# mmaker/c-lwe-snarks

Hardware: AMD Instinct MI355X
Metric: snark_proofs_per_sec (higher is better)
Workload: dtype u32 limbs (704-bit integers mod 2^704) + AES-256 bytes; int8 digits on the matrix cores, int32 accumulation (exact)

## Files before the change

### c-lwe-snarks_amd/__init__.py

```python
from __future__ import annotations

import ctypes
import os
from dataclasses import dataclass

import numpy as np

_HERE = os.path.dirname(os.path.abspath(__file__))
LIB_PATH = os.environ.get("MFHIP_LIB") or os.path.join(_HERE, "libmfhip.so")
P = 0xFFFFFFFB


class MfhError(RuntimeError):
    pass


@dataclass(frozen=True)
class Params:

    n: int = 1470
    logq: int = 736
    d: int = 1 << 15
    m: int = 21845

# ... 34 lines not shown
        return 2 * self.ctr_ct * self.d + self.ctr_ct

    @property
    def ct_limbs(self):
        return (self.n + 1) * self.L


DEBUG = Params(d=256, m=64)
DEFAULT = Params()


class _CParams(ctypes.Structure):
    _fields_ = [("n", ctypes.c_uint32), ("logq", ctypes.c_uint32), ("d", ctypes.c_uint32), ("m", ctypes.c_uint32)]


_lib = None

EXPORTS = [
    "mfh_ctx_create", "mfh_ctx_destroy", "mfh_set_stream", "mfh_sync", "mfh_scrub_staging", "mfh_last_error", "mfh_set_seed",
    "mfh_keystream", "mfh_sample_rows", "mfh_ct_add", "mfh_ct_mul_ui", "mfh_ct_addmul_ui", "mfh_eval_rows",
    "mfh_encrypt_rows", "mfh_decrypt", "mfh_ct_smudge", "mfh_ssp_upload", "mfh_witness_poly", "mfh_version",
    "mfh_workspace_bytes", "mfh_last_kernel_ms", "mfh_set_timing", "mfh_set_overlap", "mfh_eval_rows_multi", "mfh_prove_batch", "mfh_crs_mm_image_bytes", "mfh_crs_expand_mm", "mfh_crs_set_resident_mm", "mfh_witness_poly_multi", "mfh_witness_poly_mm", "mfh_poly_h_multi", "mfh_poly_mul", "mfh_poly_add", "mfh_poly_prepare_t",
    "mfh_ssp_prepare", "mfh_poly_h", "mfh_setup_messages", "mfh_setup", "mfh_setup_image", "mfh_crs_image_set_b", "mfh_prove",
    "mfh_prove_partial", "mfh_prove_finish", "mfh_ct_to_lanes", "mfh_ct_from_lanes", "mfh_lanes_per_value", "mfh_digest128", "mfh_timing_drain", "mfh_timing_busy_ms", "mfh_timing_work_rows", "mfh_set_batch_image", "mfh_set_batch_slabs", "mfh_set_expand_path", "mfh_set_encrypt_path", "mfh_set_batch_launch", "mfh_set_batch_bw", "mfh_set_mm_chunk_rows", "mfh_set_mm_pack", "mfh_set_poly_exact", "mfh_poly_exact_fallbacks", "mfh_poly_exact_points", "mfh_set_poly_exact_points", "mfh_set_mm_stream", "mfh_add_dotp", "mfh_set_encrypt_chunks", "mfh_set_witness_per", "mfh_set_eval_path", "mfh_set_decrypt_path", "mfh_decrypt_rows",
    "mfh_crs_mm_share_bytes", "mfh_crs_expand_mm_share", "mfh_crs_set_resident_mm_share", "mfh_batch_chain", "mfh_batch_witness_cols", "mfh_batch_chain_from_w", "mfh_witness_poly_mm_cols", "mfh_prove_batch_partial", "mfh_prove_batch_finish",
    "mfh_resident_row_bytes", "mfh_crs_expand", "mfh_eval_rows_resident", "mfh_crs_set_resident",
    "mfh_witness_lanes", "mfh_witness_from_lanes", "mfh_prove_partial_w", "mfh_verify",
    "mfh_ssp_set_prg", "mfh_ssp_prg_make_t", "mfh_ssp_prg_fill",
    "mfh_resident_share_rows", "mfh_crs_expand_share", "mfh_crs_set_resident_share", "mfh_crs_set_resident_prefix",
    "mfh_prove_batch_supergroup", "mfh_prove_batch_stream_wait", "mfh_set_mm_width",
    "mfh_setup_public", "mfh_prove_public", "mfh_prove_batch_public", "mfh_vk_derive", "mfh_verify_public",
    "mfh_ssp_from_rows", "mfh_ssp_set_rows", "mfh_ssp_rows_fill", "mfh_circuit_create", "mfh_circuit_destroy", "mfh_circuit_assign",
    "mfh_circuit_create_global", "mfh_circuit_create_ex", "mfh_circuit_create_out", "mfh_circuit_create_sum",
]


def load_library():
    global _lib
    if _lib is not None:
        return _lib
    if not os.path.exists(LIB_PATH):
        raise MfhError(f"{LIB_PATH} is missing: run `python -c 'import __graft_entry__ as g; g.build()'` "
                       "(hipcc --offload-arch=gfx950).  There is no CPU fallback.")
    lib = ctypes.CDLL(LIB_PATH)
    vp, u64, sz, i32, u32 = ctypes.c_void_p, ctypes.c_uint64, ctypes.c_size_t, ctypes.c_int, ctypes.c_uint32
    sig = {
        "mfh_ctx_create": (i32, [ctypes.POINTER(vp), i32, ctypes.POINTER(_CParams)]),
# ... 58 lines not shown
        "mfh_witness_from_lanes": (i32, [vp, vp, vp, u32, vp]),
        "mfh_prove_partial_w": (i32, [vp, vp, vp, ctypes.c_char_p, u32, u32, u32, vp, vp]),
        "mfh_resident_row_bytes": (sz, [vp]),
        "mfh_crs_expand": (i32, [vp, u64, sz, vp, vp]),
        "mfh_crs_image_set_b": (i32, [vp, sz, sz, vp, vp]),
        "mfh_eval_rows_resident": (i32, [vp, vp, sz, sz, vp, vp, vp, vp, i32]),
        "mfh_crs_set_resident": (i32, [vp, vp]),
        "mfh_timing_drain": (i32, [vp, ctypes.c_char_p, ctypes.POINTER(u64), ctypes.POINTER(ctypes.c_double), ctypes.POINTER(u64),
                                   ctypes.POINTER(ctypes.c_float)]),
        "mfh_timing_busy_ms": (ctypes.c_double, [vp]),
        "mfh_timing_work_rows": (u64, [vp]),
        "mfh_set_batch_image": (i32, [vp, i32]),
        "mfh_set_mm_chunk_rows": (i32, [vp, u32]),
        "mfh_set_mm_pack": (i32, [vp, i32]),
        "mfh_set_poly_exact": (i32, [vp, i32]),
        "mfh_poly_exact_fallbacks": (ctypes.c_long, [vp]),
        "mfh_poly_exact_points": (i32, [vp, ctypes.POINTER(u32)]),
        "mfh_set_poly_exact_points": (i32, [vp, ctypes.POINTER(u32)]),
        "mfh_set_mm_stream": (i32, [vp, i32, i32, i32, u32]),
        "mfh_set_batch_launch": (i32, [vp, u32, i32]),
        "mfh_set_batch_bw": (i32, [vp, i32]),
        "mfh_set_encrypt_path": (i32, [vp, i32]),
        "mfh_set_expand_path": (i32, [vp, i32]),
        "mfh_set_batch_slabs": (i32, [vp, u32]),
        "mfh_set_encrypt_chunks": (i32, [vp, u32]),
        "mfh_set_eval_path": (i32, [vp, i32]),
        "mfh_set_decrypt_path": (i32, [vp, i32]),
        "mfh_decrypt_rows": (i32, [vp, u64, sz, vp, vp, vp]),
        "mfh_set_witness_per": (i32, [vp, u32]),
        "mfh_crs_mm_share_bytes": (sz, [vp, u32, u32]),
        "mfh_crs_expand_mm_share": (i32, [vp, vp, u32, u32, vp]),
        "mfh_crs_set_resident_mm_share": (i32, [vp, vp, u32, u32]),
        "mfh_batch_chain": (i32, [vp, vp, u32, ctypes.c_char_p, sz, vp, vp, vp, vp]),
        "mfh_batch_witness_cols": (i32, [vp, vp, u32, ctypes.c_char_p, sz, vp, u32, u32, vp, sz]),
        "mfh_batch_chain_from_w": (i32, [vp, vp, u32, vp, vp, vp]),
        "mfh_witness_poly_mm_cols": (i32, [vp, vp, u32, ctypes.c_char_p, sz, vp, u32, u32, vp, sz]),
        "mfh_prove_batch_partial": (i32, [vp, vp, u32, u32, u32, ctypes.c_char_p, sz, vp, vp, vp, sz, vp]),
        "mfh_prove_batch_finish": (i32, [vp, vp, u32, vp, ctypes.c_char_p, sz, ctypes.c_char_p, vp]),
        "mfh_setup_public": (i32, [vp, vp, u32, u32, u32, u32, vp, vp, vp, vp]),
        "mfh_prove_public": (i32, [vp, vp, vp, u32, ctypes.c_char_p, u32, ctypes.c_char_p, sz, ctypes.c_char_p, vp]),
        "mfh_prove_batch_public": (i32, [vp, vp, vp, u32, u32, ctypes.c_char_p, sz, vp, ctypes.c_char_p, sz, ctypes.c_char_p, vp]),
        "mfh_vk_derive": (i32, [vp, vp, u32, u32, vp]),
        "mfh_verify_public": (i32, [vp, vp, u32, u32, u32, vp, vp, ctypes.c_char_p, sz, sz, vp]),
        "mfh_ssp_from_rows": (i32, [vp, u32, vp, vp, vp, vp]),
        "mfh_ssp_set_rows": (i32, [vp, u32, vp, vp, vp, u32]),
        "mfh_ssp_rows_fill": (i32, [vp, sz, sz, vp]),
# ... 118 lines not shown
    def scrub_staging(self):
        rc = self.lib.mfh_scrub_staging(self._h)
        self._chk(rc)
        return rc

    def workspace_bytes(self):
        return int(self.lib.mfh_workspace_bytes(self._h))

    def set_timing(self, on=True):
        self._chk(self.lib.mfh_set_timing(self._h, 1 if on else 0))

    def set_overlap(self, mode=1):
        self._chk(self.lib.mfh_set_overlap(self._h, int(mode)))

    def set_batch_image(self, on=True):
        self._chk(self.lib.mfh_set_batch_image(self._h, 1 if on else 0))

    def set_batch_slabs(self, nslabs=0):
        self._chk(self.lib.mfh_set_batch_slabs(self._h, int(nslabs)))

    def set_expand_path(self, path=0):
        self._chk(self.lib.mfh_set_expand_path(self._h, int(path)))

    def set_encrypt_path(self, path=0):
        self._chk(self.lib.mfh_set_encrypt_path(self._h, int(path)))

    def set_eval_path(self, path=0):
        self._chk(self.lib.mfh_set_eval_path(self._h, int(path)))

    def set_encrypt_chunks(self, chunks=0):
        self._chk(self.lib.mfh_set_encrypt_chunks(self._h, int(chunks)))

    def set_witness_per(self, statements=0):
        self._chk(self.lib.mfh_set_witness_per(self._h, int(statements)))

    def set_batch_launch(self, groups_per_launch=4, merge_regions=True):
        self._chk(self.lib.mfh_set_batch_launch(self._h, int(groups_per_launch), 1 if merge_regions else 0))

    def set_batch_bw(self, merged=True):
        self._chk(self.lib.mfh_set_batch_bw(self._h, 1 if merged else 0))

    def set_mm_stream(self, map=0, persistent=False, sync_mode=0, spin_max=64):
        self._chk(self.lib.mfh_set_mm_stream(self._h, int(map), int(persistent), int(sync_mode), int(spin_max)))

    def set_mm_width(self, per_xcd=32, early_chain=False):
        self._chk(self.lib.mfh_set_mm_width(self._h, int(per_xcd), 1 if early_chain else 0))
# ... 494 lines not shown
```

### c-lwe-snarks_amd/csrc/ctx.hpp

```cpp
#pragma once
#include <hip/hip_runtime.h>

#include <stdint.h>
#include <string.h>

#include <string>
#include <vector>

#include "aes_dev.hpp"
#include "mfhip.h"
#include "ssp_prg.hpp"

#define HIP_TRY(ctx, expr)                                                        \
  do {                                                                            \
    hipError_t e_ = (expr);                                                       \
    if (e_ != hipSuccess) {                                                       \
      (ctx)->err = std::string(#expr) + ": " + hipGetErrorString(e_);             \
      return MFH_EDEVICE;                                                         \
    }                                                                             \
  } while (0)

struct PolyState;
struct SspInterp;
struct SspRows;
// ... 62 lines not shown
  size_t mm_base[3] = {0, 0, 0};
  DevBuf ssp_frag;
  const uint32_t *ssp_frag_src = nullptr;
  SspInterp *interp = nullptr;
  DevBuf circ_io;
  DevBuf circ_state;
  DevBuf d_batch;
  DevBuf batch_img;
  int batch_image = 1;
  int mm_map = 1;
  bool mm_persist = true;
  bool mm_wave1 = false;
  uint32_t mm_sync_mode = 0, mm_spin = 64;
  uint32_t mm_width = 32;
  size_t early_ws_half = 0;
  bool batch_early_chain = false;
  uint32_t *mm_sync = nullptr;
  int poly_exact = 1;
  bool poly_pts_pinned = false;
  uint32_t poly_pts[4] = {0, 0, 0, 0};
  bool mm_pack = true;
  uint32_t mm_chunk_rows = 131071;
  int expand_path = 0;
  int enc_path = 0;
  uint32_t ncu = 256;
  int dec_path = 0;
  int eval_path = 0;
  uint32_t enc_chunks = 0;
  uint32_t witness_per = 0;
  uint32_t batch_slabs = 0;
  int batch_bw_merged = 1;
  int batch_merge = 1;
  uint32_t batch_ngl = 8;
  PinBuf pin_rows, pin_cw, pin_smudge;
  PinBuf pin_pub;
  DevBuf d_pub;
  PinBuf pin_wring[8];
  uint32_t pin_wnext = 0;
  hipEvent_t ev_sample = nullptr;
  DevBuf sample_tmp;
  void *uploader = nullptr;
  bool prg_on = false;
  uint64_t prg_seed = 0;
  const uint32_t *prg_t = nullptr;
  SspRows *rows = nullptr;
  RowsTree *rows_tree = nullptr;
// ... 117 lines not shown
  }
  if (!c->prg_on || !c->prg_t) { c->err = "d_ssp is NULL and no generator-defined SSP is registered (mfh_ssp_set_prg)"; return MFH_EINVAL; }
  src = mf::SspSrc{nullptr, c->prg_t, c->prg_seed};
  return MFH_OK;
}

void mfh_poly_destroy(mfh_ctx *c);
void ssp_interp_free(mfh_ctx *c);
void ssp_rows_free(mfh_ctx *c, bool tree);
int ssp_rows_check(mfh_ctx *c, const char *who, uint32_t nrows, const uint32_t *h_row_ptr, const uint32_t *h_wire, const uint32_t *h_coef);
int ssp_rows_tree(mfh_ctx *c, const char *who, const uint32_t *&d_t, const uint32_t *&h_w);
int ssp_rows_witness(mfh_ctx *c, uint32_t nstmt, const uint8_t *h_bits, size_t bits_stride, const uint32_t *h_delta, uint32_t *d_w, size_t w_stride);
int ssp_rows_msg_evals(mfh_ctx *c, uint32_t s, uint32_t beta, uint32_t *d_msg_evals);
inline bool ssp_is_rows(const mfh_ctx *c, const uint32_t *d_ssp) { return !d_ssp && c->rows_prefix; }
inline int ssp_rows_lu_check(mfh_ctx *c, const uint32_t *d_ssp, uint32_t lu) {
  if (ssp_is_rows(c, d_ssp) && lu > c->rows_lu_max) { c->err = "lu exceeds the lu_max the row SSP was registered with (mfh_ssp_set_rows)"; return MFH_EINVAL; }
  return MFH_OK;
}
extern "C" int mfh_witness_poly_mm(mfh_ctx *c, const uint32_t *d_ssp, uint32_t nstmt, const uint8_t *h_bits, size_t bits_stride, const uint32_t *h_delta,
                                   uint32_t *d_w);
extern "C" int mfh_witness_poly_mm_cols(mfh_ctx *c, const uint32_t *d_ssp, uint32_t nstmt, const uint8_t *h_bits, size_t bits_stride, const uint32_t *h_delta,
                                        uint32_t col0, uint32_t ncols, uint32_t *d_w, size_t w_stride);
extern "C" int mfh_poly_h_multi(mfh_ctx *c, const uint32_t *d_v, uint32_t *d_h, uint32_t nb);
int expand_mm_region(mfh_ctx *c, uint64_t off, uint32_t nrows, const uint8_t *c8, uint8_t *image);
int encrypt_rows_mm(mfh_ctx *c, uint64_t off, size_t nrows, const uint64_t *sk, const uint32_t *msg, const uint64_t *err, uint8_t *c8);
int decrypt_mm(mfh_ctx *c, const uint64_t *sk, const uint64_t *cts, size_t count, uint32_t *out);
int decrypt_rows_mm(mfh_ctx *c, uint64_t off, size_t nrows, const uint64_t *sk, const uint8_t *c8, uint32_t *out);

struct MmIo {
  const uint32_t *coef[2];
  uint32_t csplit;
  uint64_t *out[2];
  uint32_t osplit;
  uint64_t ostride;
  const uint8_t *bits;
  uint32_t bits_stride;
  int64_t *sc_zeroed;
  uint64_t cstride;
  uint32_t bits_row0;
  const uint64_t *add_ct;
  const uint32_t *add_scale;
  uint32_t sa_from1;
};
int eval_rows_multi_io(mfh_ctx *c, uint64_t off, size_t nrows, const uint8_t *d_c8, const MmIo &io, uint32_t nvec, uint32_t coeff_bytes, int accumulate);
int eval_rows_multi_io_set(mfh_ctx *c, uint64_t off, size_t nrows, const uint8_t *d_c8, const MmIo *ios, const uint32_t *nvecs, uint32_t ng,
                           uint32_t coeff_bytes);
struct MmRegion { uint64_t off; const uint8_t *c8; };
// ... 18 lines not shown
```

### c-lwe-snarks_amd/csrc/evalmm.hip

```cpp
#include <algorithm>
#include <cstring>

#include "ctx.hpp"

namespace {

using mf::AesKey;

constexpr int CT = 4;
constexpr int SB = 88;
constexpr int VB = 92;
constexpr int MB = CT * SB;
constexpr int MT = MB / 32;
constexpr int RT = 128;
constexpr int TSTRIDE = 384;
constexpr int BLK_PER_ROW = 24;
static_assert(MB % 32 == 0 && CT * VB + 15 <= TSTRIDE, "tile geometry");

typedef int v4i __attribute__((ext_vector_type(4)));
typedef int v16i __attribute__((ext_vector_type(16)));

__device__ __forceinline__ uint32_t coef_at(const MmIo &io, uint32_t v, uint32_t nrows, uint32_t i) {
  if (io.bits) {
    const uint32_t a = io.bits_row0 + i;
// ... 1613 lines not shown
  const uint64_t d = c->P.d, m = c->P.m;
  const uint64_t loS = d * rank / world, cS = d * (rank + 1) / world - loS, lo = m * rank / world, cnt = m * (rank + 1) / world - lo;
  return MmShare{{loS, d + loS, 2 * d + lo}, {cS, cS, cnt}};
}
size_t mfh_crs_mm_share_bytes(const mfh_ctx *c, uint32_t rank, uint32_t world) {
  if (!c || !world || rank >= world) return 0;
  const MmShare sh = mm_share(c, rank, world);
  return mm_region_bytes(c, sh.rows[0]) + mm_region_bytes(c, sh.rows[1]) + mm_region_bytes(c, sh.rows[2]);
}
size_t mfh_crs_mm_image_bytes(const mfh_ctx *c) { return mfh_crs_mm_share_bytes(c, 0, 1); }
int mfh_crs_expand_mm_share(mfh_ctx *c, const uint8_t *d_crs_c8, uint32_t rank, uint32_t world, uint8_t *d_image) {
  if (!c || !d_crs_c8 || !d_image || !world || rank >= world) return MFH_EINVAL;
  if (!c->have_seed) { c->err = "mfh_set_seed has not been called"; return MFH_EINVAL; }
  const WideGeom wg = wide_geom(c);
  const uint32_t n = c->P.n;
  if (((uint64_t)n * wg.vby) & 7) { c->err = "mfh_crs_expand_mm: the row length must be a multiple of 8"; return MFH_EUNSUPPORTED; }
  HIP_TRY(c, hipSetDevice(c->device));
  const uint64_t ctr_ct = (uint64_t)wg.vby * n;
  const MmShare sh = mm_share(c, rank, world);
  AesKey keyx = c->key;
  for (int i = 56; i < 60; i++) keyx.rk[i] ^= 0x80808080u;
  const uint32_t ntiles = (n + 1 + wg.ct - 1) / wg.ct;
  size_t base = 0;
  for (int r = 0; r < 3; r++) {
    if (!sh.rows[r]) continue;
    const uint32_t units = (uint32_t)((sh.rows[r] + RT2 - 1) / RT2);
    const uint32_t nchunks = std::max(1u, std::min(units, 4u));
    const uint32_t rpc = (units + nchunks - 1) / nchunks * RT2;
    Timer t(c, 9, sh.rows[r]);
    const dim3 grid(ntiles, (uint32_t)((sh.rows[r] + rpc - 1) / rpc));
    const uint8_t *c8 = d_crs_c8 + (size_t)sh.row0[r] * wg.vby;
    if (c->expand_path == 0 && ((ctr_ct * sh.row0[r]) & 7) == 0) {
      int rc = expand_mm_region(c, ctr_ct * sh.row0[r], (uint32_t)sh.rows[r], c8, d_image + base);
      if (rc) return rc;
      base += mm_region_bytes(c, sh.rows[r]);
      continue;
    }
    if (c->P.logq == 736)
      hipLaunchKernelGGL((k_evalmm16<1, 736>), grid, dim3(1024), 0, c->stream, keyx, c->d_t0, ctr_ct * sh.row0[r], n, (uint32_t)sh.rows[r], rpc, c8,
                         (const int8_t *)nullptr, (int *)nullptr, d_image + base);
    else
      hipLaunchKernelGGL((k_evalmm16<1, 1472>), grid, dim3(1024), 0, c->stream, keyx, c->d_t0, ctr_ct * sh.row0[r], n, (uint32_t)sh.rows[r], rpc, c8,
                         (const int8_t *)nullptr, (int *)nullptr, d_image + base);
    base += mm_region_bytes(c, sh.rows[r]);
  }
  HIP_TRY(c, hipGetLastError());
  return MFH_OK;
}
int mfh_crs_expand_mm(mfh_ctx *c, const uint8_t *d_crs_c8, uint8_t *d_image) { return mfh_crs_expand_mm_share(c, d_crs_c8, 0, 1, d_image); }
int mfh_set_mm_stream(mfh_ctx *c, int map, int persistent, int sync_mode, uint32_t spin_max) {
  if (!c || map < 0 || map > 1 || sync_mode < 0 || sync_mode > 2 || persistent < 0 || persistent > 2) return MFH_EINVAL;
  c->mm_map = map;
  c->mm_persist = persistent != 0;
  c->mm_wave1 = persistent == 2;
  c->mm_sync_mode = (uint32_t)sync_mode;
  c->mm_spin = spin_max;
  return MFH_OK;
}
int mfh_set_mm_width(mfh_ctx *c, uint32_t per_xcd, int early_chain) {
  if (!c || per_xcd < 1 || per_xcd > 32) return MFH_EINVAL;
  c->mm_width = per_xcd;
  c->batch_early_chain = early_chain != 0;
  return MFH_OK;
}
int mfh_set_mm_pack(mfh_ctx *c, int on) {
  if (!c) return MFH_EINVAL;
  c->mm_pack = on != 0;
  return MFH_OK;
// ... 123 lines not shown
```

### c-lwe-snarks_amd/csrc/expandmm.hip

```cpp
#include <algorithm>

#include "ctx.hpp"

namespace {

using mf::AesKey;
typedef int v4i __attribute__((ext_vector_type(4)));

constexpr uint32_t PADW = 0x80808080u;
constexpr int MACB = 23;

template <int LOGQ> struct XG;
template <> struct XG<736> { static constexpr int DW = 23, SIG = 22, CPM = 4, PPM = 22, MT = 11, CT = 2; };
template <> struct XG<1472> { static constexpr int DW = 46, SIG = 46, CPM = 2, PPM = 24, MT = 12, CT = 1; };

struct Plan {
  int nemit;
  int src[2][4];
  int piece[2];
  int npend;
  int pend[3];
};
template <int LOGQ>
constexpr Plan make_plan(int T) {
  using G = XG<LOGQ>;
  int np = 0, piece = 0;
  Plan cur{};
  for (int t = 0; t <= T; t++) {
    int list[8] = {7, 7, 7, 7, 7, 7, 7, 7}, nl = 0;
    for (int i = 0; i < np; i++) list[nl++] = i;
// ... 2 lines not shown
      const int within = (4 * t + i) % G::DW;
      if (within < G::SIG) list[nl++] = 3 + i;
      if (nl == 4 || (LOGQ == 1472 && within == G::DW - 1 && nl > 0)) {
        for (int k = 0; k < 4; k++) cur.src[cur.nemit][k] = k < nl ? list[k] : 7;
        cur.piece[cur.nemit] = piece++;
        cur.nemit++;
        nl = 0;
      }
    }
    cur.npend = nl;
    for (int k = 0; k < 3; k++) cur.pend[k] = k < nl ? list[k] : 7;
    np = nl;
  }
  return cur;
}
static_assert(make_plan<736>(22).npend == 0 && make_plan<736>(22).piece[make_plan<736>(22).nemit - 1] == 21, "22 pieces per period at logq 736");
static_assert(make_plan<1472>(22).npend == 0 && make_plan<1472>(22).nemit == 2 && make_plan<1472>(22).piece[1] == 23, "24 pieces per period at logq 1472");
static_assert(make_plan<736>(5).nemit == 0 && make_plan<736>(5).npend == 3 && make_plan<736>(6).nemit == 1 && make_plan<736>(6).npend == 3, "the block holding a value's insignificant dword yields 3 dwords");

__device__ __forceinline__ uint32_t pick(int code, const uint32_t (&p)[3], const uint32_t (&v)[4]) {
  return code < 3 ? p[code] : code < 7 ? v[code - 3] : PADW;
}

template <int LOGQ>
__global__ __launch_bounds__(1024) __attribute__((amdgpu_waves_per_eu(8, 8))) void k_expand_mm(
    AesKey key , const uint32_t *__restrict__ g_t0, uint64_t off, uint32_t n, uint32_t nrows,
    uint32_t periods_per_chunk, const uint8_t *__restrict__ c8, v4i *__restrict__ image, uint32_t KS, uint32_t mtiles) {
  using G = XG<LOGQ>;
  __shared__ __attribute__((aligned(16))) uint32_t lt[mf::kTabBytes / 4];
  mf::lds_fill_tab(lt, g_t0);
  const uint8_t *tab = reinterpret_cast<const uint8_t *>(lt);
  const mf::AesLane L = mf::aes_lane();
  const uint32_t lane = threadIdx.x & 63;
  const uint32_t wave = __builtin_amdgcn_readfirstlane(threadIdx.x >> 6);
  const uint32_t ks = blockIdx.y * 16 + wave;
  const uint32_t row = 64 * ks + lane;
  const uint32_t rowdw = n * G::DW;
  const uint32_t nper = (n + 1 + G::CPM - 1) / G::CPM;
  const uint32_t m0 = blockIdx.x * periods_per_chunk, m1 = min(nper, m0 + periods_per_chunk);
  __syncthreads();
  if (64 * ks >= nrows || m0 >= m1) return;
  const uint64_t rowstart = off + (uint64_t)row * rowdw * 4;
  const bool shifted = (rowstart & 8) != 0;
  const uint32_t *__restrict__ bw = reinterpret_cast<const uint32_t *>(c8 + (uint64_t)min(row, nrows - 1) * (G::DW * 4));
  const uint32_t c16 = lane & 15, g4 = lane >> 4;
  const uint32_t one = 1u << (8 * (c16 & 3));
  const v4i selb = {(int)((c16 >> 2) == 0 ? one : 0u), (int)((c16 >> 2) == 1 ? one : 0u), (int)((c16 >> 2) == 2 ? one : 0u), (int)((c16 >> 2) == 3 ? one : 0u)};
  auto emit = [&](uint32_t P, uint32_t d0, uint32_t d1, uint32_t d2, uint32_t d3) {
    asm volatile("" : "+s"(P));
    const v4i a = {(int)d0, (int)d1, (int)d2, (int)d3};
    const v4i zero = {0, 0, 0, 0};
    uint32_t w[4];
#pragma unroll
    for (int s = 0; s < 4; s++) {
      const bool mine = g4 == (uint32_t)s;
      const v4i bs = {mine ? selb[0] : 0, mine ? selb[1] : 0, mine ? selb[2] : 0, mine ? selb[3] : 0};
      const v4i d = __builtin_amdgcn_mfma_i32_16x16x64_i8(a, bs, zero, 0, 0, 0);
      const uint32_t lo = __builtin_amdgcn_perm((uint32_t)d[1], (uint32_t)d[0], 0x0c0c0400u);
      const uint32_t hi = __builtin_amdgcn_perm((uint32_t)d[3], (uint32_t)d[2], 0x04000c0cu);
      w[s] = lo | hi;
    }
    {
      auto r02 = __builtin_amdgcn_permlane32_swap(w[0], w[2], false, false);
      auto r13 = __builtin_amdgcn_permlane32_swap(w[1], w[3], false, false);
      auto r01 = __builtin_amdgcn_permlane16_swap(r02[0], r13[0], false, false);
      auto r23 = __builtin_amdgcn_permlane16_swap(r02[1], r13[1], false, false);
      w[0] = r01[0]; w[1] = r01[1]; w[2] = r23[0]; w[3] = r23[1];
    }
    if (P < mtiles) {
      char *frag = reinterpret_cast<char *>(image) + ((uint64_t)P * KS + ks) * 1024;
      uint32_t z = 0;
      asm volatile("" : "+s"(z));
      const uint32_t l16 = __builtin_amdgcn_mbcnt_hi(~0u, __builtin_amdgcn_mbcnt_lo(~0u, z)) << 4;
      *reinterpret_cast<v4i *>(frag + l16) = v4i{(int)w[0], (int)w[1], (int)w[2], (int)w[3]};
    }
  };

  const uint64_t cb0 = rowstart >> 4;
  uint64_t ctr = cb0 + (uint64_t)m0 * MACB;
  const uint64_t span_a = ctr >> 8;
  uint32_t sca[5], scb[5];
#ifdef MF_AES_GL_EXPAND
  const mf::AesGl GLT = mf::aes_gl(g_t0 + 256);
#endif
  mf::aes_span_consts(tab, L, key, span_a, sca);
  mf::aes_span_consts(tab, L, key, span_a + 1, scb);
  auto block = [&](uint64_t c, uint32_t (&o)[4]) {
    const bool crossed = (c >> 8) != span_a;
    uint32_t sc[5];
#pragma unroll
    for (int i = 0; i < 5; i++) sc[i] = crossed ? scb[i] : sca[i];
#ifdef MF_AES_GL_EXPAND
    mf::aes256_ctr_block_sc<true>(tab, L, key, c, sc, o, &GLT);
#else
    mf::aes256_ctr_block_sc(tab, L, key, c, sc, o);
#endif
  };
  uint32_t x[4];
  block(ctr, x);
  uint32_t pend[3] = {PADW, PADW, PADW};
  for (uint32_t m = m0; m < m1; m++) {
    const uint32_t pbase = m * G::PPM;
    const uint32_t qbase = m * (MACB * 4);
#pragma unroll 1
    for (uint32_t t = 0; t < (uint32_t)MACB; t++) {
      const uint32_t q0 = qbase + 4 * t;
      uint32_t v[4];
      if (q0 < rowdw) {
        ctr++;
        uint32_t y[4];
        block(ctr, y);
        v[0] = shifted ? x[2] : x[0];
        v[1] = shifted ? x[3] : x[1];
        v[2] = shifted ? y[0] : x[2];
        v[3] = shifted ? y[1] : x[3];
#pragma unroll
        for (int i = 0; i < 4; i++) x[i] = y[i];
      } else {
#pragma unroll
        for (int i = 0; i < 4; i++) v[i] = PADW;
      }
      if (q0 + 3 >= rowdw) {
#pragma unroll
        for (int i = 0; i < 4; i++) {
          const uint32_t q = q0 + i;
          if (q >= rowdw) v[i] = q - rowdw < (uint32_t)G::DW ? bw[q - rowdw] ^ PADW : PADW;
        }
      }
      switch (t) {
#define XCASE(T)                                                                                                                        \
  case T: {                                                                                                                             \
    constexpr Plan pl = make_plan<LOGQ>(T);                                                                                             \
    const uint32_t p0[3] = {pend[0], pend[1], pend[2]};                                                                                 \
    if constexpr (pl.nemit >= 1) emit(pbase + pl.piece[0], pick(pl.src[0][0], p0, v), pick(pl.src[0][1], p0, v), pick(pl.src[0][2], p0, v), pick(pl.src[0][3], p0, v)); \
    if constexpr (pl.nemit >= 2) emit(pbase + pl.piece[1], pick(pl.src[1][0], p0, v), pick(pl.src[1][1], p0, v), pick(pl.src[1][2], p0, v), pick(pl.src[1][3], p0, v)); \
    pend[0] = pick(pl.pend[0], p0, v);                                                                                                  \
    pend[1] = pick(pl.pend[1], p0, v);                                                                                                  \
    pend[2] = pick(pl.pend[2], p0, v);                                                                                                  \
  } break;
        XCASE(0) XCASE(1) XCASE(2) XCASE(3) XCASE(4) XCASE(5) XCASE(6) XCASE(7) XCASE(8) XCASE(9) XCASE(10) XCASE(11) XCASE(12) XCASE(13) XCASE(14) XCASE(15)
        XCASE(16) XCASE(17) XCASE(18) XCASE(19) XCASE(20) XCASE(21) XCASE(22)
#undef XCASE
        default: break;
      }
    }
  }
}

}

int expand_mm_region(mfh_ctx *c, uint64_t off, uint32_t nrows, const uint8_t *c8, uint8_t *image) {
  const uint32_t n = c->P.n;
  const bool q736 = c->P.logq == 736;
  const uint32_t ct = q736 ? XG<736>::CT : XG<1472>::CT, mt = q736 ? XG<736>::MT : XG<1472>::MT, cpm = q736 ? XG<736>::CPM : XG<1472>::CPM;
  const uint32_t mtiles = (n + 1 + ct - 1) / ct * mt;
  const uint32_t KS = (nrows + 255) / 256 * 4;
  const uint32_t ksteps = (nrows + 63) / 64, nper = (n + 1 + cpm - 1) / cpm;
  const uint32_t gy = (ksteps + 15) / 16;
  uint32_t ppc = 10;
  while (ppc > 2 && (uint64_t)gy * ((nper + ppc - 1) / ppc) < 4096) ppc--;
  const uint32_t gx = (nper + ppc - 1) / ppc;
  mf::AesKey keyx = c->key;
  for (int i = 56; i < 60; i++) keyx.rk[i] ^= 0x80808080u;
  if (q736)
    hipLaunchKernelGGL(k_expand_mm<736>, dim3(gx, gy), dim3(1024), 0, c->stream, keyx, c->d_t0, off, n, nrows, ppc, c8, (v4i *)image, KS, mtiles);
  else
    hipLaunchKernelGGL(k_expand_mm<1472>, dim3(gx, gy), dim3(1024), 0, c->stream, keyx, c->d_t0, off, n, nrows, ppc, c8, (v4i *)image, KS, mtiles);
  return MFH_OK;
}
```

### c-lwe-snarks_amd/csrc/mfhip.hip

```cpp
#include <hip/hip_runtime.h>

#include <stdint.h>
#include <stdio.h>
#include <string.h>

#include <algorithm>
#include <string>
#include <thread>
#include <vector>

#include "aes_dev.hpp"
#include "mfhip.h"

using mf::AesKey;

template <int LOGQ>
struct PS {
  static constexpr int CTB = LOGQ / 8;
  static constexpr int EW = CTB / 4;
  static constexpr int L = (LOGQ + 63) / 64;
  static constexpr int K = LOGQ / 64;
  static constexpr int KW = 2 * K;
  static constexpr int TILE = LOGQ == 736 ? 512 : 256;
  static constexpr int ROWS = 2;
// ... 1014 lines not shown
  if (!c) return MFH_EINVAL;
  pin_scrub(c->pin_rows);
  pin_scrub(c->pin_cw);
  pin_scrub(c->pin_smudge);
  for (auto &b : c->pin_wring) pin_scrub(b);
  return MFH_OK;
}

const char *mfh_last_error(const mfh_ctx *c) { return c ? c->err.c_str() : "null context"; }
size_t mfh_workspace_bytes(const mfh_ctx *c) { return c ? c->ws.cap : 0; }
int mfh_set_overlap(mfh_ctx *c, int en) {
  if (!c) return MFH_EINVAL;
  c->overlap = en != 0;
  c->overlap_mode = en > 1 ? en : 1;
  return MFH_OK;
}

int mfh_set_expand_path(mfh_ctx *c, int path) {
  if (!c || path < 0 || path > 1) return MFH_EINVAL;
  c->expand_path = path;
  return MFH_OK;
}

int mfh_set_encrypt_path(mfh_ctx *c, int path) {
  if (!c || path < 0 || path > 2) return MFH_EINVAL;
  c->enc_path = path;
  return MFH_OK;
}

int mfh_set_eval_path(mfh_ctx *c, int path) {
  if (!c || path < 0 || path > 1) return MFH_EINVAL;
  c->eval_path = path;
  return MFH_OK;
}
int mfh_set_encrypt_chunks(mfh_ctx *c, uint32_t chunks) {
  if (!c || chunks > 64) return MFH_EINVAL;
  c->enc_chunks = chunks;
  return MFH_OK;
}
int mfh_set_witness_per(mfh_ctx *c, uint32_t statements) {
  if (!c || (statements && (statements < 32 || statements > 256))) return MFH_EINVAL;
  c->witness_per = statements;
  return MFH_OK;
}
int mfh_set_batch_slabs(mfh_ctx *c, uint32_t nslabs) {
  if (!c || nslabs > 256) return MFH_EINVAL;
// ... 835 lines not shown
```

### include/mfhip.h

```cpp
#pragma once
#include <stddef.h>
#include <stdint.h>

#ifdef __cplusplus
extern "C" {
#endif

#define MFH_P 0xfffffffbu

enum {
  MFH_OK = 0,
  MFH_EINVAL = -1,
  MFH_EDEVICE = -2,
  MFH_ENOMEM = -3,
  MFH_EUNSUPPORTED = -4
};

typedef struct {
  uint32_t n;
  uint32_t logq;
  uint32_t d;
  uint32_t m;
} mfh_params;

// ... 98 lines not shown
int mfh_setup_image(mfh_ctx *ctx, const uint32_t *d_ssp, uint32_t alpha, uint32_t beta, uint32_t s, const uint64_t *d_sk,
                    const uint64_t *d_err, uint8_t *d_crs_c8, void *d_rows_image);
int mfh_prove(mfh_ctx *ctx, const uint8_t *d_crs_c8, const uint32_t *d_ssp, const uint8_t *h_witness_bits, uint32_t delta,
              const uint8_t *h_smudge_mag, size_t maglen, const uint8_t *h_smudge_sign, uint64_t *d_proof);

int mfh_verify(mfh_ctx *ctx, const uint32_t *d_ssp, uint32_t alpha, uint32_t beta, uint32_t s, const uint64_t *d_sk,
               const uint64_t *d_proofs, size_t count, uint8_t *d_ok);

int mfh_setup_public(mfh_ctx *ctx, const uint32_t *d_ssp, uint32_t alpha, uint32_t beta, uint32_t s, uint32_t lu, const uint64_t *d_sk,
                     const uint64_t *d_err, uint8_t *d_crs_c8, void *d_rows_image);
int mfh_prove_public(mfh_ctx *ctx, const uint8_t *d_crs_c8, const uint32_t *d_ssp, uint32_t lu, const uint8_t *h_bits, uint32_t delta,
                     const uint8_t *h_smudge_mag, size_t maglen, const uint8_t *h_smudge_sign, uint64_t *d_proof);
int mfh_prove_batch_public(mfh_ctx *ctx, const uint8_t *d_crs_c8, const uint32_t *d_ssp, uint32_t lu, uint32_t nproofs, const uint8_t *h_bits,
                           size_t bits_stride, const uint32_t *h_delta, const uint8_t *h_smudge_mag, size_t maglen, const uint8_t *h_smudge_sign,
                           uint64_t *d_proofs);
int mfh_vk_derive(mfh_ctx *ctx, const uint32_t *d_ssp, uint32_t s, uint32_t lu, uint32_t *d_vk);
int mfh_verify_public(mfh_ctx *ctx, const uint32_t *d_vk, uint32_t lu, uint32_t alpha, uint32_t beta, const uint64_t *d_sk, const uint64_t *d_proofs,
                      const uint8_t *h_statements, size_t stmt_stride, size_t count, uint8_t *d_ok);

size_t mfh_crs_mm_image_bytes(const mfh_ctx *ctx);
int mfh_crs_expand_mm(mfh_ctx *ctx, const uint8_t *d_crs_c8, uint8_t *d_image);
int mfh_crs_set_resident_mm(mfh_ctx *ctx, const uint8_t *d_image);
int mfh_set_expand_path(mfh_ctx *ctx, int path);
int mfh_set_batch_image(mfh_ctx *ctx, int enabled);
int mfh_set_batch_slabs(mfh_ctx *ctx, uint32_t nslabs);
int mfh_set_encrypt_chunks(mfh_ctx *ctx, uint32_t chunks);
int mfh_set_eval_path(mfh_ctx *ctx, int path);
int mfh_set_witness_per(mfh_ctx *ctx, uint32_t statements);
int mfh_set_batch_launch(mfh_ctx *ctx, uint32_t groups_per_launch, int merge_regions);
int mfh_set_batch_bw(mfh_ctx *ctx, int merged);
int mfh_set_mm_stream(mfh_ctx *ctx, int map, int persistent, int sync_mode, uint32_t spin_max);
int mfh_set_mm_width(mfh_ctx *ctx, uint32_t per_xcd, int early_chain);
int mfh_set_mm_chunk_rows(mfh_ctx *ctx, uint32_t rows);
int mfh_set_mm_pack(mfh_ctx *ctx, int on);
int mfh_prove_batch(mfh_ctx *ctx, const uint8_t *d_crs_c8, const uint32_t *d_ssp, uint32_t nproofs, const uint8_t *h_witness_bits,
                    size_t bits_stride, const uint32_t *h_delta, const uint8_t *h_smudge_mag, size_t maglen, const uint8_t *h_smudge_sign,
                    uint64_t *d_proofs);
uint32_t mfh_prove_batch_supergroup(const mfh_ctx *ctx);
int mfh_prove_batch_stream_wait(mfh_ctx *ctx, uint32_t upto, void *hip_stream);
size_t mfh_crs_mm_share_bytes(const mfh_ctx *ctx, uint32_t rank, uint32_t world);
int mfh_crs_expand_mm_share(mfh_ctx *ctx, const uint8_t *d_crs_c8, uint32_t rank, uint32_t world, uint8_t *d_image);
int mfh_crs_set_resident_mm_share(mfh_ctx *ctx, const uint8_t *d_image, uint32_t rank, uint32_t world);
int mfh_batch_chain(mfh_ctx *ctx, const uint32_t *d_ssp, uint32_t nstmt, const uint8_t *h_witness_bits, size_t bits_stride, const uint32_t *h_delta,
                    uint32_t *d_w, uint32_t *d_h, uint32_t *d_v);
int mfh_batch_witness_cols(mfh_ctx *ctx, const uint32_t *d_ssp, uint32_t nstmt, const uint8_t *h_witness_bits, size_t bits_stride, const uint32_t *h_delta,
                           uint32_t col0, uint32_t ncols, uint32_t *d_w, size_t w_stride);
// ... 40 lines not shown
```

Baseline: 13940.

## Merge CRS expand regions into one persistent launch with LDS transpose staging

```diff
diff --git a/c-lwe-snarks_amd/__init__.py b/c-lwe-snarks_amd/__init__.py
--- a/c-lwe-snarks_amd/__init__.py
+++ b/c-lwe-snarks_amd/__init__.py
@@ -80,7 +80,7 @@
     "mfh_encrypt_rows", "mfh_decrypt", "mfh_ct_smudge", "mfh_ssp_upload", "mfh_witness_poly", "mfh_version",
     "mfh_workspace_bytes", "mfh_last_kernel_ms", "mfh_set_timing", "mfh_set_overlap", "mfh_eval_rows_multi", "mfh_prove_batch", "mfh_crs_mm_image_bytes", "mfh_crs_expand_mm", "mfh_crs_set_resident_mm", "mfh_witness_poly_multi", "mfh_witness_poly_mm", "mfh_poly_h_multi", "mfh_poly_mul", "mfh_poly_add", "mfh_poly_prepare_t",
     "mfh_ssp_prepare", "mfh_poly_h", "mfh_setup_messages", "mfh_setup", "mfh_setup_image", "mfh_crs_image_set_b", "mfh_prove",
-    "mfh_prove_partial", "mfh_prove_finish", "mfh_ct_to_lanes", "mfh_ct_from_lanes", "mfh_lanes_per_value", "mfh_digest128", "mfh_timing_drain", "mfh_timing_busy_ms", "mfh_timing_work_rows", "mfh_set_batch_image", "mfh_set_batch_slabs", "mfh_set_expand_path", "mfh_set_encrypt_path", "mfh_set_batch_launch", "mfh_set_batch_bw", "mfh_set_mm_chunk_rows", "mfh_set_mm_pack", "mfh_set_poly_exact", "mfh_poly_exact_fallbacks", "mfh_poly_exact_points", "mfh_set_poly_exact_points", "mfh_set_mm_stream", "mfh_add_dotp", "mfh_set_encrypt_chunks", "mfh_set_witness_per", "mfh_set_eval_path", "mfh_set_decrypt_path", "mfh_decrypt_rows",
+    "mfh_prove_partial", "mfh_prove_finish", "mfh_ct_to_lanes", "mfh_ct_from_lanes", "mfh_lanes_per_value", "mfh_digest128", "mfh_timing_drain", "mfh_timing_busy_ms", "mfh_timing_work_rows", "mfh_set_batch_image", "mfh_set_batch_slabs", "mfh_set_expand_path", "mfh_set_expand_run", "mfh_set_encrypt_path", "mfh_set_batch_launch", "mfh_set_batch_bw", "mfh_set_mm_chunk_rows", "mfh_set_mm_pack", "mfh_set_poly_exact", "mfh_poly_exact_fallbacks", "mfh_poly_exact_points", "mfh_set_poly_exact_points", "mfh_set_mm_stream", "mfh_add_dotp", "mfh_set_encrypt_chunks", "mfh_set_witness_per", "mfh_set_eval_path", "mfh_set_decrypt_path", "mfh_decrypt_rows",
     "mfh_crs_mm_share_bytes", "mfh_crs_expand_mm_share", "mfh_crs_set_resident_mm_share", "mfh_batch_chain", "mfh_batch_witness_cols", "mfh_batch_chain_from_w", "mfh_witness_poly_mm_cols", "mfh_prove_batch_partial", "mfh_prove_batch_finish",
     "mfh_resident_row_bytes", "mfh_crs_expand", "mfh_eval_rows_resident", "mfh_crs_set_resident",
     "mfh_witness_lanes", "mfh_witness_from_lanes", "mfh_prove_partial_w", "mfh_verify",
@@ -185,6 +185,7 @@
         "mfh_set_batch_bw": (i32, [vp, i32]),
         "mfh_set_encrypt_path": (i32, [vp, i32]),
         "mfh_set_expand_path": (i32, [vp, i32]),
+        "mfh_set_expand_run": (i32, [vp, i32]),
         "mfh_set_batch_slabs": (i32, [vp, u32]),
         "mfh_set_encrypt_chunks": (i32, [vp, u32]),
         "mfh_set_eval_path": (i32, [vp, i32]),
@@ -349,6 +350,9 @@
     def set_expand_path(self, path=0):
         self._chk(self.lib.mfh_set_expand_path(self._h, int(path)))
 
+    def set_expand_run(self, periods=0):
+        self._chk(self.lib.mfh_set_expand_run(self._h, int(periods)))
+
     def set_encrypt_path(self, path=0):
         self._chk(self.lib.mfh_set_encrypt_path(self._h, int(path)))
 
diff --git a/c-lwe-snarks_amd/csrc/ctx.hpp b/c-lwe-snarks_amd/csrc/ctx.hpp
--- a/c-lwe-snarks_amd/csrc/ctx.hpp
+++ b/c-lwe-snarks_amd/csrc/ctx.hpp
@@ -108,6 +108,7 @@
   bool mm_pack = true;
   uint32_t mm_chunk_rows = 131071;
   int expand_path = 0;
+  int expand_run = 0;
   int enc_path = 0;
   uint32_t ncu = 256;
   int dec_path = 0;
@@ -271,7 +272,8 @@
 extern "C" int mfh_witness_poly_mm_cols(mfh_ctx *c, const uint32_t *d_ssp, uint32_t nstmt, const uint8_t *h_bits, size_t bits_stride, const uint32_t *h_delta,
                                         uint32_t col0, uint32_t ncols, uint32_t *d_w, size_t w_stride);
 extern "C" int mfh_poly_h_multi(mfh_ctx *c, const uint32_t *d_v, uint32_t *d_h, uint32_t nb);
-int expand_mm_region(mfh_ctx *c, uint64_t off, uint32_t nrows, const uint8_t *c8, uint8_t *image);
+struct ExpandRegion { uint64_t off; uint32_t nrows; const uint8_t *c8; uint8_t *image; };
+int expand_mm_regions(mfh_ctx *c, const ExpandRegion *regs, int nreg);
 int encrypt_rows_mm(mfh_ctx *c, uint64_t off, size_t nrows, const uint64_t *sk, const uint32_t *msg, const uint64_t *err, uint8_t *c8);
 int decrypt_mm(mfh_ctx *c, const uint64_t *sk, const uint64_t *cts, size_t count, uint32_t *out);
 int decrypt_rows_mm(mfh_ctx *c, uint64_t off, size_t nrows, const uint64_t *sk, const uint8_t *c8, uint32_t *out);
diff --git a/c-lwe-snarks_amd/csrc/evalmm.hip b/c-lwe-snarks_amd/csrc/evalmm.hip
--- a/c-lwe-snarks_amd/csrc/evalmm.hip
+++ b/c-lwe-snarks_amd/csrc/evalmm.hip
@@ -1659,20 +1659,21 @@
   for (int i = 56; i < 60; i++) keyx.rk[i] ^= 0x80808080u;
   const uint32_t ntiles = (n + 1 + wg.ct - 1) / wg.ct;
   size_t base = 0;
+  ExpandRegion fast[3];
+  int nfast = 0;
   for (int r = 0; r < 3; r++) {
     if (!sh.rows[r]) continue;
+    const uint8_t *c8 = d_crs_c8 + (size_t)sh.row0[r] * wg.vby;
+    if (c->expand_path == 0 && ((ctr_ct * sh.row0[r]) & 7) == 0) {
+      fast[nfast++] = ExpandRegion{ctr_ct * sh.row0[r], (uint32_t)sh.rows[r], c8, d_image + base};
+      base += mm_region_bytes(c, sh.rows[r]);
+      continue;
+    }
     const uint32_t units = (uint32_t)((sh.rows[r] + RT2 - 1) / RT2);
     const uint32_t nchunks = std::max(1u, std::min(units, 4u));
     const uint32_t rpc = (units + nchunks - 1) / nchunks * RT2;
     Timer t(c, 9, sh.rows[r]);
     const dim3 grid(ntiles, (uint32_t)((sh.rows[r] + rpc - 1) / rpc));
-    const uint8_t *c8 = d_crs_c8 + (size_t)sh.row0[r] * wg.vby;
-    if (c->expand_path == 0 && ((ctr_ct * sh.row0[r]) & 7) == 0) {
-      int rc = expand_mm_region(c, ctr_ct * sh.row0[r], (uint32_t)sh.rows[r], c8, d_image + base);
-      if (rc) return rc;
-      base += mm_region_bytes(c, sh.rows[r]);
-      continue;
-    }
     if (c->P.logq == 736)
       hipLaunchKernelGGL((k_evalmm16<1, 736>), grid, dim3(1024), 0, c->stream, keyx, c->d_t0, ctr_ct * sh.row0[r], n, (uint32_t)sh.rows[r], rpc, c8,
                          (const int8_t *)nullptr, (int *)nullptr, d_image + base);
@@ -1681,6 +1682,8 @@
                          (const int8_t *)nullptr, (int *)nullptr, d_image + base);
     base += mm_region_bytes(c, sh.rows[r]);
   }
+  if (nfast)
+    if (int rc = expand_mm_regions(c, fast, nfast)) return rc;
   HIP_TRY(c, hipGetLastError());
   return MFH_OK;
 }
diff --git a/c-lwe-snarks_amd/csrc/expandmm.hip b/c-lwe-snarks_amd/csrc/expandmm.hip
--- a/c-lwe-snarks_amd/csrc/expandmm.hip
+++ b/c-lwe-snarks_amd/csrc/expandmm.hip
@@ -6,6 +6,12 @@
 
 using mf::AesKey;
 typedef int v4i __attribute__((ext_vector_type(4)));
+typedef int v2i __attribute__((ext_vector_type(2)));
+typedef __attribute__((address_space(3))) v2i lds_v2i;
+typedef __attribute__((address_space(3))) v4i lds_v4i;
+typedef __attribute__((address_space(3))) char lds_char;
+typedef __attribute__((address_space(1))) v4i glb_v4i;
+typedef __attribute__((address_space(1))) char glb_char;
 
 constexpr uint32_t PADW = 0x80808080u;
 constexpr int MACB = 23;
@@ -54,126 +60,139 @@
   return code < 3 ? p[code] : code < 7 ? v[code - 3] : PADW;
 }
 
+constexpr int MAXREG = 3;
+constexpr uint32_t kMinRun = 12;
+struct XRegions {
+  uint64_t off[MAXREG];
+  const uint8_t *c8[MAXREG];
+  v4i *image[MAXREG];
+  uint32_t nrows[MAXREG];
+  uint32_t ks_end[MAXREG];
+};
+
+__device__ __forceinline__ uint32_t stage_write_offset(uint32_t lane) { return ((lane & 0x30) << 3) | ((lane & 8) << 6) | ((lane & 7) << 4); }
+
 template <int LOGQ>
 __global__ __launch_bounds__(1024) __attribute__((amdgpu_waves_per_eu(8, 8))) void k_expand_mm(
-    AesKey key , const uint32_t *__restrict__ g_t0, uint64_t off, uint32_t n, uint32_t nrows,
-    uint32_t periods_per_chunk, const uint8_t *__restrict__ c8, v4i *__restrict__ image, uint32_t KS, uint32_t mtiles) {
+    AesKey key , const uint32_t *__restrict__ g_t0, XRegions R, uint32_t n, uint32_t mtiles,
+    uint32_t units, uint32_t units_q, uint32_t units_r , uint32_t run_max) {
   using G = XG<LOGQ>;
-  __shared__ __attribute__((aligned(16))) uint32_t lt[mf::kTabBytes / 4];
+  __shared__ __attribute__((aligned(16))) uint32_t lt[(mf::kTabBytes + 16 * 1024) / 4];
   mf::lds_fill_tab(lt, g_t0);
   const uint8_t *tab = reinterpret_cast<const uint8_t *>(lt);
   const mf::AesLane L = mf::aes_lane();
   const uint32_t lane = threadIdx.x & 63;
   const uint32_t wave = __builtin_amdgcn_readfirstlane(threadIdx.x >> 6);
-  const uint32_t ks = blockIdx.y * 16 + wave;
-  const uint32_t row = 64 * ks + lane;
   const uint32_t rowdw = n * G::DW;
   const uint32_t nper = (n + 1 + G::CPM - 1) / G::CPM;
-  const uint32_t m0 = blockIdx.x * periods_per_chunk, m1 = min(nper, m0 + periods_per_chunk);
+  uint8_t *const stage = reinterpret_cast<uint8_t *>(lt) + mf::kTabBytes + 1024 * wave;
+  uint32_t st_w = (uint32_t)(uintptr_t)(lds_char *)(stage + stage_write_offset(lane));
+  uint32_t st_r = (uint32_t)(uintptr_t)(lds_char *)(stage + 8 * lane);
+  asm volatile("" : "+v"(st_w), "+v"(st_r));
+  const uint32_t l16 = lane << 4;
+  const uint32_t gw = wave * gridDim.x + blockIdx.x;
+  uint32_t u = (uint32_t)min((uint64_t)units, (uint64_t)units_q * gw + min(gw, units_r));
+  const uint32_t u_end = (uint32_t)min((uint64_t)units, (uint64_t)u + units_q + (gw < units_r ? 1u : 0u));
   __syncthreads();
-  if (64 * ks >= nrows || m0 >= m1) return;
-  const uint64_t rowstart = off + (uint64_t)row * rowdw * 4;
-  const bool shifted = (rowstart & 8) != 0;
-  const uint32_t *__restrict__ bw = reinterpret_cast<const uint32_t *>(c8 + (uint64_t)min(row, nrows - 1) * (G::DW * 4));
-  const uint32_t c16 = lane & 15, g4 = lane >> 4;
-  const uint32_t one = 1u << (8 * (c16 & 3));
-  const v4i selb = {(int)((c16 >> 2) == 0 ? one : 0u), (int)((c16 >> 2) == 1 ? one : 0u), (int)((c16 >> 2) == 2 ? one : 0u), (int)((c16 >> 2) == 3 ? one : 0u)};
-  auto emit = [&](uint32_t P, uint32_t d0, uint32_t d1, uint32_t d2, uint32_t d3) {
-    asm volatile("" : "+s"(P));
-    const v4i a = {(int)d0, (int)d1, (int)d2, (int)d3};
-    const v4i zero = {0, 0, 0, 0};
-    uint32_t w[4];
-#pragma unroll
-    for (int s = 0; s < 4; s++) {
-      const bool mine = g4 == (uint32_t)s;
-      const v4i bs = {mine ? selb[0] : 0, mine ? selb[1] : 0, mine ? selb[2] : 0, mine ? selb[3] : 0};
-      const v4i d = __builtin_amdgcn_mfma_i32_16x16x64_i8(a, bs, zero, 0, 0, 0);
-      const uint32_t lo = __builtin_amdgcn_perm((uint32_t)d[1], (uint32_t)d[0], 0x0c0c0400u);
-      const uint32_t hi = __builtin_amdgcn_perm((uint32_t)d[3], (uint32_t)d[2], 0x04000c0cu);
-      w[s] = lo | hi;
-    }
-    {
-      auto r02 = __builtin_amdgcn_permlane32_swap(w[0], w[2], false, false);
-      auto r13 = __builtin_amdgcn_permlane32_swap(w[1], w[3], false, false);
-      auto r01 = __builtin_amdgcn_permlane16_swap(r02[0], r13[0], false, false);
-      auto r23 = __builtin_amdgcn_permlane16_swap(r02[1], r13[1], false, false);
-      w[0] = r01[0]; w[1] = r01[1]; w[2] = r23[0]; w[3] = r23[1];
-    }
-    if (P < mtiles) {
-      char *frag = reinterpret_cast<char *>(image) + ((uint64_t)P * KS + ks) * 1024;
-      uint32_t z = 0;
-      asm volatile("" : "+s"(z));
-      const uint32_t l16 = __builtin_amdgcn_mbcnt_hi(~0u, __builtin_amdgcn_mbcnt_lo(~0u, z)) << 4;
-      *reinterpret_cast<v4i *>(frag + l16) = v4i{(int)w[0], (int)w[1], (int)w[2], (int)w[3]};
-    }
-  };
-
-  const uint64_t cb0 = rowstart >> 4;
-  uint64_t ctr = cb0 + (uint64_t)m0 * MACB;
-  const uint64_t span_a = ctr >> 8;
-  uint32_t sca[5], scb[5];
 #ifdef MF_AES_GL_EXPAND
   const mf::AesGl GLT = mf::aes_gl(g_t0 + 256);
 #endif
-  mf::aes_span_consts(tab, L, key, span_a, sca);
-  mf::aes_span_consts(tab, L, key, span_a + 1, scb);
-  auto block = [&](uint64_t c, uint32_t (&o)[4]) {
-    const bool crossed = (c >> 8) != span_a;
-    uint32_t sc[5];
-#pragma unroll
-    for (int i = 0; i < 5; i++) sc[i] = crossed ? scb[i] : sca[i];
+  while (u < u_end) {
+    const uint32_t kg = u / nper, m0 = u - kg * nper;
+    uint32_t m1 = min(nper, m0 + (u_end - u));
+    if (run_max) m1 = min(m1, m0 + run_max);
+    u += m1 - m0;
+    const uint32_t reg = (kg >= R.ks_end[0] ? 1u : 0u) + (kg >= R.ks_end[1] ? 1u : 0u);
+    const uint32_t ks_first = reg ? R.ks_end[reg - 1] : 0u;
+    const uint32_t ks = kg - ks_first, KS = R.ks_end[reg] - ks_first;
+    const uint32_t nrows = R.nrows[reg];
+    const bool live = 64 * ks < nrows;
+    const uint32_t row = 64 * ks + lane;
+    const uint64_t rowstart = R.off[reg] + (uint64_t)row * rowdw * 4;
+    const bool shifted = (rowstart & 8) != 0;
+    const uint32_t *__restrict__ bw = reinterpret_cast<const uint32_t *>(R.c8[reg] + (uint64_t)min(row, nrows - 1) * (G::DW * 4));
+    const uint32_t ksdw = live ? rowdw : 0u;
+    const uint32_t bdw = live ? rowdw : 0xfffffff0u;
+    const uint32_t fstride = KS * 1024;
+    uint64_t fcur = reinterpret_cast<uint64_t>(R.image[reg]) + (uint64_t)ks * 1024 + (uint64_t)(m0 * G::PPM) * fstride;
+    int32_t fleft = (int32_t)mtiles - (int32_t)(m0 * G::PPM);
+    auto emit = [&](uint32_t d0, uint32_t d1, uint32_t d2, uint32_t d3) {
+      *(lds_v4i *)(uintptr_t)st_w = v4i{(int)d0, (int)d1, (int)d2, (int)d3};
+      const v2i lo = __builtin_amdgcn_ds_read_tr8_b64_v2i32((lds_v2i *)(uintptr_t)st_r);
+      const v2i hi = __builtin_amdgcn_ds_read_tr8_b64_v2i32((lds_v2i *)(uintptr_t)st_r + 64);
+      asm volatile("" : "+s"(fcur));
+      uint32_t lo16 = l16;
+      asm volatile("" : "+v"(lo16));
+      if (fleft > 0) *reinterpret_cast<glb_v4i *>(reinterpret_cast<glb_char *>(fcur) + lo16) = v4i{lo[0], lo[1], hi[0], hi[1]};
+      fcur += fstride;
+      fleft--;
+    };
+
+    uint64_t ctr = (rowstart >> 4) + (uint64_t)m0 * MACB;
+    uint32_t sc[5], scn[5];
+    auto block = [&](uint64_t c, uint32_t (&o)[4]) {
 #ifdef MF_AES_GL_EXPAND
-    mf::aes256_ctr_block_sc<true>(tab, L, key, c, sc, o, &GLT);
+      mf::aes256_ctr_block_sc<true>(tab, L, key, c, sc, o, &GLT);
 #else
-    mf::aes256_ctr_block_sc(tab, L, key, c, sc, o);
+      mf::aes256_ctr_block_sc(tab, L, key, c, sc, o);
 #endif
-  };
-  uint32_t x[4];
-  block(ctr, x);
-  uint32_t pend[3] = {PADW, PADW, PADW};
-  for (uint32_t m = m0; m < m1; m++) {
-    const uint32_t pbase = m * G::PPM;
-    const uint32_t qbase = m * (MACB * 4);
+    };
+    uint32_t x[4] = {PADW, PADW, PADW, PADW};
+    if (live) {
+      mf::aes_span_consts(tab, L, key, ctr >> 8, sc);
+      mf::aes_span_consts(tab, L, key, (ctr >> 8) + 1, scn);
+      block(ctr, x);
+    }
+    uint32_t pend[3] = {PADW, PADW, PADW};
+    for (uint32_t m = m0; m < m1; m++) {
+      const uint32_t qbase = m * (MACB * 4);
+      if (live && m != m0 && ((m - m0) & 7) == 0) mf::aes_span_consts(tab, L, key, (ctr >> 8) + 1, scn);
 #pragma unroll 1
-    for (uint32_t t = 0; t < (uint32_t)MACB; t++) {
-      const uint32_t q0 = qbase + 4 * t;
-      uint32_t v[4];
-      if (q0 < rowdw) {
-        ctr++;
-        uint32_t y[4];
-        block(ctr, y);
-        v[0] = shifted ? x[2] : x[0];
-        v[1] = shifted ? x[3] : x[1];
-        v[2] = shifted ? y[0] : x[2];
-        v[3] = shifted ? y[1] : x[3];
-#pragma unroll
-        for (int i = 0; i < 4; i++) x[i] = y[i];
-      } else {
-#pragma unroll
-        for (int i = 0; i < 4; i++) v[i] = PADW;
-      }
-      if (q0 + 3 >= rowdw) {
-#pragma unroll
-        for (int i = 0; i < 4; i++) {
-          const uint32_t q = q0 + i;
-          if (q >= rowdw) v[i] = q - rowdw < (uint32_t)G::DW ? bw[q - rowdw] ^ PADW : PADW;
+      for (uint32_t t = 0; t < (uint32_t)MACB; t++) {
+        const uint32_t q0 = qbase + 4 * t;
+        uint32_t v[4];
+        if (q0 < ksdw) {
+          ctr++;
+          const bool cross = ((uint32_t)ctr & 255u) == 0;
+          if (__builtin_amdgcn_ballot_w64(cross)) {
+#pragma unroll
+            for (int i = 0; i < 5; i++) sc[i] = cross ? scn[i] : sc[i];
+          }
+          uint32_t y[4];
+          block(ctr, y);
+          v[0] = shifted ? x[2] : x[0];
+          v[1] = shifted ? x[3] : x[1];
+          v[2] = shifted ? y[0] : x[2];
+          v[3] = shifted ? y[1] : x[3];
+#pragma unroll
+          for (int i = 0; i < 4; i++) x[i] = y[i];
+        } else {
+#pragma unroll
+          for (int i = 0; i < 4; i++) v[i] = PADW;
         }
-      }
-      switch (t) {
+        if (q0 + 3 >= bdw) {
+#pragma unroll
+          for (int i = 0; i < 4; i++) {
+            const uint32_t q = q0 + i;
+            if (q >= rowdw) v[i] = q - rowdw < (uint32_t)G::DW ? bw[q - rowdw] ^ PADW : PADW;
+          }
+        }
+        switch (t) {
 #define XCASE(T)                                                                                                                        \
   case T: {                                                                                                                             \
     constexpr Plan pl = make_plan<LOGQ>(T);                                                                                             \
     const uint32_t p0[3] = {pend[0], pend[1], pend[2]};                                                                                 \
-    if constexpr (pl.nemit >= 1) emit(pbase + pl.piece[0], pick(pl.src[0][0], p0, v), pick(pl.src[0][1], p0, v), pick(pl.src[0][2], p0, v), pick(pl.src[0][3], p0, v)); \
-    if constexpr (pl.nemit >= 2) emit(pbase + pl.piece[1], pick(pl.src[1][0], p0, v), pick(pl.src[1][1], p0, v), pick(pl.src[1][2], p0, v), pick(pl.src[1][3], p0, v)); \
+    if constexpr (pl.nemit >= 1) emit(pick(pl.src[0][0], p0, v), pick(pl.src[0][1], p0, v), pick(pl.src[0][2], p0, v), pick(pl.src[0][3], p0, v)); \
+    if constexpr (pl.nemit >= 2) emit(pick(pl.src[1][0], p0, v), pick(pl.src[1][1], p0, v), pick(pl.src[1][2], p0, v), pick(pl.src[1][3], p0, v)); \
     pend[0] = pick(pl.pend[0], p0, v);                                                                                                  \
     pend[1] = pick(pl.pend[1], p0, v);                                                                                                  \
     pend[2] = pick(pl.pend[2], p0, v);                                                                                                  \
   } break;
-        XCASE(0) XCASE(1) XCASE(2) XCASE(3) XCASE(4) XCASE(5) XCASE(6) XCASE(7) XCASE(8) XCASE(9) XCASE(10) XCASE(11) XCASE(12) XCASE(13) XCASE(14) XCASE(15)
-        XCASE(16) XCASE(17) XCASE(18) XCASE(19) XCASE(20) XCASE(21) XCASE(22)
+          XCASE(0) XCASE(1) XCASE(2) XCASE(3) XCASE(4) XCASE(5) XCASE(6) XCASE(7) XCASE(8) XCASE(9) XCASE(10) XCASE(11) XCASE(12) XCASE(13) XCASE(14) XCASE(15)
+          XCASE(16) XCASE(17) XCASE(18) XCASE(19) XCASE(20) XCASE(21) XCASE(22)
 #undef XCASE
-        default: break;
+          default: break;
+        }
       }
     }
   }
@@ -181,22 +200,39 @@
 
 }
 
-int expand_mm_region(mfh_ctx *c, uint64_t off, uint32_t nrows, const uint8_t *c8, uint8_t *image) {
+int expand_mm_regions(mfh_ctx *c, const ExpandRegion *regs, int nreg) {
   const uint32_t n = c->P.n;
   const bool q736 = c->P.logq == 736;
   const uint32_t ct = q736 ? XG<736>::CT : XG<1472>::CT, mt = q736 ? XG<736>::MT : XG<1472>::MT, cpm = q736 ? XG<736>::CPM : XG<1472>::CPM;
   const uint32_t mtiles = (n + 1 + ct - 1) / ct * mt;
-  const uint32_t KS = (nrows + 255) / 256 * 4;
-  const uint32_t ksteps = (nrows + 63) / 64, nper = (n + 1 + cpm - 1) / cpm;
-  const uint32_t gy = (ksteps + 15) / 16;
-  uint32_t ppc = 10;
-  while (ppc > 2 && (uint64_t)gy * ((nper + ppc - 1) / ppc) < 4096) ppc--;
-  const uint32_t gx = (nper + ppc - 1) / ppc;
+  const uint32_t nper = (n + 1 + cpm - 1) / cpm;
   mf::AesKey keyx = c->key;
   for (int i = 56; i < 60; i++) keyx.rk[i] ^= 0x80808080u;
-  if (q736)
-    hipLaunchKernelGGL(k_expand_mm<736>, dim3(gx, gy), dim3(1024), 0, c->stream, keyx, c->d_t0, off, n, nrows, ppc, c8, (v4i *)image, KS, mtiles);
-  else
-    hipLaunchKernelGGL(k_expand_mm<1472>, dim3(gx, gy), dim3(1024), 0, c->stream, keyx, c->d_t0, off, n, nrows, ppc, c8, (v4i *)image, KS, mtiles);
+  const uint32_t nwg = 2 * c->ncu, waves = 16 * nwg;
+  for (int r0 = 0; r0 < nreg; r0 += MAXREG) {
+    XRegions R{};
+    uint64_t ksteps = 0;
+    uint32_t rows = 0;
+    for (int i = 0; i < MAXREG; i++) {
+      if (r0 + i < nreg) {
+        const ExpandRegion &g = regs[r0 + i];
+        R.off[i] = g.off; R.c8[i] = g.c8; R.image[i] = reinterpret_cast<v4i *>(g.image); R.nrows[i] = g.nrows;
+        ksteps += (g.nrows + 255) / 256 * 4;
+        rows += g.nrows;
+      }
+      R.ks_end[i] = (uint32_t)ksteps;
+    }
+    const uint64_t units = ksteps * nper;
+    if (!units) continue;
+    if (units >> 32) { c->err = "mfh_crs_expand_mm: too many rows for one launch"; return MFH_EUNSUPPORTED; }
+    Timer t(c, 9, rows);
+    uint32_t uq = (uint32_t)(units / waves), ur = (uint32_t)(units % waves);
+    if (uq < kMinRun) { uq = kMinRun; ur = 0; }
+    const uint32_t run = (uint32_t)c->expand_run;
+    if (q736)
+      hipLaunchKernelGGL(k_expand_mm<736>, dim3(nwg), dim3(1024), 0, c->stream, keyx, c->d_t0, R, n, mtiles, (uint32_t)units, uq, ur, run);
+    else
+      hipLaunchKernelGGL(k_expand_mm<1472>, dim3(nwg), dim3(1024), 0, c->stream, keyx, c->d_t0, R, n, mtiles, (uint32_t)units, uq, ur, run);
+  }
   return MFH_OK;
 }
diff --git a/c-lwe-snarks_amd/csrc/mfhip.hip b/c-lwe-snarks_amd/csrc/mfhip.hip
--- a/c-lwe-snarks_amd/csrc/mfhip.hip
+++ b/c-lwe-snarks_amd/csrc/mfhip.hip
@@ -1060,6 +1060,12 @@
   return MFH_OK;
 }
 
+int mfh_set_expand_run(mfh_ctx *c, int periods) {
+  if (!c || periods < 0) return MFH_EINVAL;
+  c->expand_run = periods;
+  return MFH_OK;
+}
+
 int mfh_set_encrypt_path(mfh_ctx *c, int path) {
   if (!c || path < 0 || path > 2) return MFH_EINVAL;
   c->enc_path = path;
diff --git a/include/mfhip.h b/include/mfhip.h
--- a/include/mfhip.h
+++ b/include/mfhip.h
@@ -144,6 +144,7 @@
 int mfh_crs_expand_mm(mfh_ctx *ctx, const uint8_t *d_crs_c8, uint8_t *d_image);
 int mfh_crs_set_resident_mm(mfh_ctx *ctx, const uint8_t *d_image);
 int mfh_set_expand_path(mfh_ctx *ctx, int path);
+int mfh_set_expand_run(mfh_ctx *ctx, int periods);
 int mfh_set_batch_image(mfh_ctx *ctx, int enabled);
 int mfh_set_batch_slabs(mfh_ctx *ctx, uint32_t nslabs);
 int mfh_set_encrypt_chunks(mfh_ctx *ctx, uint32_t chunks);
```

Measured after the change: 13920. No clear change (-0.1%).
